# pangenome/allwave

Measured on AMD Instinct MI355X. Metric: aligned base-pairs/sec (whole node) + PAF lines/sec, all-pairs 10 kbp, higher is better.
Workload: dtype int16

## Files before the change

allwave_amd/csrc/biwfa_device.hpp:

```cpp


#include <hip/hip_runtime.h>
#include <stdint.h>
#include <limits.h>

#include "range_span.hpp"
#include "twin_base.hpp"
#include "row_reuse.hpp"

#ifndef AWV_NS
#define AWV_NS awv
#endif
#ifndef AWV_WG
#define AWV_WG 64
#endif
namespace AWV_NS {

constexpr int WG = AWV_WG;
constexpr int MAX_SCOPE = 126;
constexpr int MAX_RING = 256;
constexpr int NCOMP = 5;
constexpr int32_t OFF_NULL = INT32_MIN / 2;
constexpr int32_t NULLISH = INT32_MIN / 4;
constexpr int32_t NULL16 = -16384;
#ifdef AWV_WIDE16
constexpr bool WENC = true;
#else
constexpr bool WENC = false;
#endif
enum { C_M = 0, C_I1 = 1, C_I2 = 2, C_D1 = 3, C_D2 = 4 };
constexpr int FALLBACK_MIN_SCORE = 250;
constexpr int FALLBACK_MIN_LENGTH = 100;
constexpr int STACK_CAP = 48;
constexpr int EV_STACK_WORDS = (STACK_CAP * 32 + 3) / 4 + 16;
constexpr int EV_TWIN_WORDS = MAX_SCOPE * NCOMP;
constexpr int SUB16_MAX_LEN = 32760;
#ifndef AWV_WAVES_PER_SIMD
#define AWV_WAVES_PER_SIMD 4
#endif
constexpr int WAVES_PER_SIMD = AWV_WAVES_PER_SIMD;
constexpr int STATIC_LDS_RESERVE = 1024;
constexpr int COL_PAD = 576;

constexpr int ST_OK = 0, ST_CAPACITY = 1, ST_INTERNAL = 2, ST_MAX_STEPS = 3, ST_ABOVE_BOUND = 4;
constexpr int ST_TWIN_REDO = 64;

struct DevPenalties {
  int x, o1, e1, o2, e2, two_piece, scope;
};

struct DevResult {
  int32_t status, penalty, score;
  uint32_t cigar_len;
  uint64_t cigar_off;
  int32_t num_matches, num_mismatches, num_ins, num_del, q_end, t_end;
};

enum { STAT_CELLS = 0, STAT_EXTEND, STAT_BREAKPOINTS, STAT_BASE, STAT_OVERLAP, STAT_ALIGNED_BP, STAT_PAIRS,
       STAT_T_TOTAL, STAT_T_BI_COMPUTE, STAT_T_BI_BARRIER, STAT_T_BI_FINALIZE, STAT_T_OVERLAP, STAT_T_BASE_STEPS,
       STAT_T_BACKTRACE, STAT_T_EMIT, STAT_N_PASSES,
       STAT_T_CR_LOAD, STAT_T_CR_ALU, STAT_T_CR_EXTEND, STAT_T_CR_STORE, STAT_T_CR_REDUCE, STAT_RESTARTS, STAT_MULTI_CELLS, STAT_WIN_SINGLE, STAT_WIN_MULTI, STAT_WIN_BASE, STAT_WIN_BASE_MULTI,
       STAT_CLK_CYCLES, STAT_CLK_TICKS,
       STAT_DEEP_CELLS,
       STAT_N,
       STAT_TWIN_UNITS = STAT_N, STAT_TWIN_SHARED, STAT_TWIN_SOLO, STAT_TWIN_NONMIRROR,
       STAT_REUSE_CELLS, STAT_REUSE_SEARCHES,
       STAT_N_DEV };

#ifdef AWV_PROF
#define PROF_DRAIN() __builtin_amdgcn_s_waitcnt(0)
#define PROF_NOW() __builtin_readcyclecounter()
#define PROF_ADD(slot, t0) do { if (threadIdx.x == 0) lstats[slot] += __builtin_readcyclecounter() - (t0); } while (0)
#define PROF_INC(slot) do { if (threadIdx.x == 0) lstats[slot] += 1; } while (0)
#define PROF_ADD_L(slot, t0) do { if (threadIdx.x == 0) sh.prof[(slot) - STAT_T_CR_LOAD] += __builtin_readcyclecounter() - (t0); } while (0)
#else
#define PROF_ADD_L(slot, t0) do { (void)(t0); } while (0)
#define PROF_DRAIN() do { } while (0)
#define PROF_NOW() 0ULL
#define PROF_ADD(slot, t0) do { (void)(t0); } while (0)
#define PROF_INC(slot) do { } while (0)
#endif

struct KParams {
  const uint8_t* seq[4];
  const uint64_t* seq_off;
  const int32_t* seq_len;
  const uint32_t* seq2[2];
  const uint64_t* seq2_off;
  const uint8_t* seq2_ok;
  const int32_t* pair_q;
  const int32_t* pair_t;
  const int32_t* pair_rc;
  long long npairs;
  DevPenalties pen;
  int ring;
  int chain_max;
  int multi_T;
  int deep_passes;
  int sub16;
  int wcap;
  void* ring_mem;
  size_t ring_slot_stride;
  int lds_meta_bytes;
  int lds_seq_bytes;
  int sb_cap;
  int wb_cap;
  void* hist_mem;
  size_t hist_slot_stride;
  size_t hist_meta_offset;
  uint32_t* ev_mem;
  size_t ev_slot_stride;
  uint8_t* cigar;
  const uint64_t* cigar_off;
  DevResult* results;
  unsigned long long* work_counter;
  unsigned long long* stats;
  int score_only;
  int max_penalty;
  const int32_t* pair_max_penalty;
  const int32_t* unit_first;
  const int32_t* unit_twin;
  int twin_levels;
  int twin_base;
};
constexpr int RR_DESC_WORDS = 4;

struct RowMeta { int lo, hi; };
constexpr int K_BIG = 1 << 28;
#define ROW_EMPTY RowMeta{K_BIG, -K_BIG}
struct Acc { int hull_lo[NCOMP]; int hull_hi[NCOMP]; int maxak; int oob; int reach; };
struct Task { int pb, pe, tb, te, cb, ce, score_remaining, known; };
constexpr int TM_A = 0, TM_B = 1, TM_SHARED = 2;
constexpr bool TWIN_BUILD = WG == 64 && !WENC;
constexpr int TWIN_MAGIC = 0x7477696e;
__device__ __forceinline__ int twin_comp(int c) { return c == 0 ? 0 : (c <= 2 ? c + 2 : c - 2); }
struct Breakpoint { int score, sf, sr, kf, kr, off_f, off_r, comp; };
static_assert(sizeof(Task) == 32 && sizeof(Breakpoint) == 32, "stack entry / twin record size");

__device__ __forceinline__ int s_min(int a, int b) { int r; asm("s_min_i32 %0, %1, %2" : "=s"(r) : "s"(a), "s"(b) : "scc"); return r; }
__device__ __forceinline__ int s_max(int a, int b) { int r; asm("s_max_i32 %0, %1, %2" : "=s"(r) : "s"(a), "s"(b) : "scc"); return r; }
__device__ __forceinline__ int s_add(int a, int b) { int r; asm("s_add_i32 %0, %1, %2" : "=s"(r) : "s"(a), "s"(b) : "scc"); return r; }

struct alignas(4) RowMeta16 { int16_t lo, hi; };
template <typename OffT> struct MetaTraits;
#ifdef AWV_WIDE16
template <> struct MetaTraits<int16_t> { typedef RowMeta Stored; };
#else
template <> struct MetaTraits<int16_t> { typedef RowMeta16 Stored; };
#endif
template <> struct MetaTraits<int32_t> { typedef RowMeta Stored; };
__device__ __forceinline__ RowMeta meta_load(const RowMeta16* p) {
  const RowMeta16 m = *p;
  return m.lo > m.hi ? ROW_EMPTY : RowMeta{m.lo, m.hi};
}
__device__ __forceinline__ RowMeta meta_load(const RowMeta* p) { return *p; }
__device__ __forceinline__ void meta_store(RowMeta16* p, const RowMeta& m) {
  *p = m.lo > m.hi ? RowMeta16{1, 0} : RowMeta16{(int16_t)m.lo, (int16_t)m.hi};
}
__device__ __forceinline__ void meta_store_scalar(RowMeta16* p, int lo, int hi) {
  int w;
  asm("s_pack_ll_b32_b16 %0, %1, %2\n\ts_cmp_gt_i32 %1, %2\n\ts_cselect_b32 %0, 1, %0" : "=&s"(w) : "s"(lo), "s"(hi) : "scc");
  *reinterpret_cast<int*>(p) = w;
}
__device__ __forceinline__ void meta_store_scalar(RowMeta* p, int lo, int hi) {
  int l, h;
  asm("s_cmp_gt_i32 %2, %3\n\ts_cselect_b32 %0, %4, %2\n\ts_cselect_b32 %1, %5, %3" : "=&s"(l), "=&s"(h) : "s"(lo), "s"(hi), "s"(K_BIG), "s"(-K_BIG) : "scc");
  *p = RowMeta{l, h};
}
__device__ __forceinline__ void meta_store(RowMeta* p, const RowMeta& m) { *p = m; }

template <typename OffT>
struct Lds {
  typename MetaTraits<OffT>::Stored* ring_meta;
  int* bi_A;
  int* bi_oob;
  int* firstk;
  uint32_t* seq;
  RowMeta* meta_log;
};
struct PassCtx {
  unsigned long long ring_mem;
  unsigned long long ring_bytes;
  unsigned long long P[2], T[2];
  int ring, wcap;
  int x, o1, e1, o2, e2;
// ... 3701 lines not shown
  cx.tb_abs = uni(pc.tb_abs);
  Lds<OffT> lds;
  typedef typename MetaTraits<OffT>::Stored MetaStored;
  lds.ring_meta = reinterpret_cast<MetaStored*>(dyn_smem);
  lds.bi_A = reinterpret_cast<int*>(lds.ring_meta + 2 * NCOMP * kp.ring);
  lds.bi_oob = lds.bi_A + 2 * kp.ring;
  lds.firstk = lds.bi_oob + 2 * kp.ring;
  lds.seq = reinterpret_cast<uint32_t*>(dyn_smem + kp.lds_meta_bytes);
  lds.meta_log = nullptr;
  void* ring_mem = (void*)(__attribute__((address_space(1))) char*)(uintptr_t)uni64(pc.ring_mem);
  const rsrc_t ring_rs = make_rsrc(ring_mem, kp.ring_slot_stride);
  __syncthreads();
  Breakpoint bp;
  const int rc = find_breakpoint_reuse<P2, OffT>(kp, sh, lds, cx, ring_mem, ring_rs, cb, ce, score_remaining, known, attempt, bp, lstats);
  if (threadIdx.x == 0) sh.bp_out = bp;
  __syncthreads();
  return rc;
}

template <bool P2, typename OffT, typename... PairSpan>
__global__ __launch_bounds__(WG, WAVES_PER_SIMD) void biwfa_align_kernel(KParams kp, PairSpan... pair_span_arg) {
  constexpr bool RANGES = sizeof...(PairSpan) > 0;
  static_assert(sizeof...(PairSpan) <= 1, "one optional argument: const awvr::Span*");
  __shared__ Shared sh;
  __shared__ unsigned long long lstats[STAT_N];
  static_assert(sizeof(Shared) + sizeof(unsigned long long) * STAT_N <= STATIC_LDS_RESERVE, "static LDS reserve");
  extern __shared__ __attribute__((aligned(16))) unsigned char dyn_smem[];
  Lds<OffT> lds;
  typedef typename MetaTraits<OffT>::Stored MetaStored;
  lds.ring_meta = reinterpret_cast<MetaStored*>(dyn_smem);
  lds.bi_A = reinterpret_cast<int*>(lds.ring_meta + 2 * NCOMP * kp.ring);
  lds.bi_oob = lds.bi_A + 2 * kp.ring;
  lds.firstk = lds.bi_oob + 2 * kp.ring;
  lds.seq = reinterpret_cast<uint32_t*>(dyn_smem + kp.lds_meta_bytes);
  const int tid = cold_tid();
  const DevPenalties& pn = kp.pen;
  void* ring_mem = (char*)kp.ring_mem + (size_t)blockIdx.x * kp.ring_slot_stride;
  void* hist = (char*)kp.hist_mem + (size_t)blockIdx.x * kp.hist_slot_stride;
  uint32_t* events = kp.ev_mem + (size_t)blockIdx.x * kp.ev_slot_stride;
  Task* const stack = reinterpret_cast<Task*>(events + kp.wcap);
  const rsrc_t hist_rs = make_rsrc(hist, kp.hist_slot_stride);
  lds.meta_log = reinterpret_cast<RowMeta*>((char*)hist + kp.hist_meta_offset);
  if (tid < STAT_N) lstats[tid] = 0;
#ifdef AWV_PROF
  if (tid < 5) sh.prof[tid] = 0;
#endif
  const unsigned long long clk_c0 = __builtin_amdgcn_s_memtime(), clk_r0 = __builtin_amdgcn_s_memrealtime();
  if (tid < 16) sh.chain_maxak[tid >> 3][tid & 7] = 0;
  __syncthreads();
  constexpr bool TWINS = TWIN_BUILD && !RANGES && sizeof(OffT) == 2;
  if constexpr (TWINS) {
  const unsigned long long rr_mem = kp.stats[STAT_N_DEV], rr_stride = kp.stats[STAT_N_DEV + 1], rr_pt = kp.stats[STAT_N_DEV + 2];
  const int rr_passes = uni((int)(unsigned)rr_pt), rr_T = uni((int)(rr_pt >> 32)), rr_nid = uni((int)kp.stats[STAT_N_DEV + 3]);
  int* const rr_hdr = rr_mem != 0 && rr_passes > 0 && pn.scope * NCOMP >= RRS_WORDS ? (int*)((char*)(uintptr_t)rr_mem + (size_t)blockIdx.x * (size_t)rr_stride) : nullptr;
  if (rr_hdr != nullptr && tid < awvrr::H_WORDS) rr_hdr[tid] = 0;
  for (;;) {
    if (tid == 0) {
      sh.cur_pair = (long long)atomicAdd(kp.work_counter, 1ULL);
      sh.win_single = sh.win_multi = sh.win_base = sh.win_base_multi = 0;
    }
    __syncthreads();
    const long long unit = ((long long)uni((int)(sh.cur_pair >> 32)) << 32) | (unsigned)uni((int)sh.cur_pair);
    if (unit >= kp.npairs) break;
    long long pair = unit, pair_b = -1;
    if constexpr (TWINS) {
      if (kp.unit_first) {
        pair = uni(kp.unit_first[unit]);
        pair_b = uni(kp.unit_twin[unit]);
      }
    }
    const int qi = kp.pair_q[pair], ti = kp.pair_t[pair];
    const int qv = kp.pair_rc[pair] ? 2 : 0;
    const uint64_t qoff = kp.seq_off[qi], toff = kp.seq_off[ti];
    int plenT = kp.seq_len[qi], tlenT = kp.seq_len[ti];
    const uint8_t* Pf = kp.seq[qv] + qoff;
    const uint8_t* Pr = kp.seq[qv + 1] + qoff;
    const uint8_t* Tf = kp.seq[0] + toff;
    const uint8_t* Tr = kp.seq[1] + toff;
    const int qok = (kp.seq2_ok[qi] >> (qv ? 1 : 0)) & 1, tok = kp.seq2_ok[ti] & 1;
    gwords_t Pw = nullptr, Tw = nullptr;
    if (qok && tok && kp.lds_seq_bytes > 0) {
      Pw = (gwords_t)(uintptr_t)(kp.seq2[qv ? 1 : 0] + kp.seq2_off[qi]);
      Tw = (gwords_t)(uintptr_t)(kp.seq2[0] + kp.seq2_off[ti]);
    }
    int tw_shared = 0, tw_solo = 0, tw_nonmirror = 0;
    int run_mode = TWINS && pair_b >= 0 ? TM_SHARED : TM_A;
    int todo = 0;
    for (;;) {
    const unsigned long long tt0 = PROF_NOW();
    int cur = TM_A;
    Emit em, em_o;
    em.cig = kp.score_only ? nullptr : kp.cigar + kp.cigar_off[pair];
    em.n = 0;
    em.cnt[0] = em.cnt[1] = em.cnt[2] = em.cnt[3] = 0;
    em_o = em;
    if (pair_b >= 0 && !kp.score_only) em_o.cig = kp.cigar + kp.cigar_off[pair_b];
    int status = ST_OK;
    int penalty = -1, penalty_o = -1;
    bool top = true, top_o = true;
    auto face = [&](int o) {
      if (cur == o) return;
      cur = o;
      { const uint8_t* x = Pf; Pf = Tf; Tf = x; }
      { const uint8_t* x = Pr; Pr = Tr; Tr = x; }
      { const gwords_t x = Pw; Pw = Tw; Tw = x; }
      { const int x = plenT; plenT = tlenT; tlenT = x; }
// ... 52 lines not shown
      cx.T[0] = to_global(Tf + t.tb);
      cx.P[1] = to_global(Pr + (plenT - t.pe));
      cx.T[1] = to_global(Tr + (tlenT - t.te));
      cx.kmin[0] = cx.kmin[1] = 0;
      cx.wcols = 0;
      cx.Pw = Pw;
      cx.Tw = Tw;
      cx.pb_abs = t.pb;
      cx.tb_abs = t.tb;
      stage_sequences<OffT>(kp, lds, cx);
      do_base = t.score_remaining <= FALLBACK_MIN_SCORE;
      if (!do_base) {
        int rc = BP_OK;
        for (int attempt = 0; attempt < AWV_RESTART_ATTEMPTS; ++attempt) {
          if (tid == 0) {
            PassCtx& pc = sh.pctx;
            pc.ring_mem = (unsigned long long)(uintptr_t)ring_mem;
            pc.ring_bytes = (unsigned long long)kp.ring_slot_stride;
            pc.P[0] = (unsigned long long)(uintptr_t)cx.P[0];
            pc.P[1] = (unsigned long long)(uintptr_t)cx.P[1];
            pc.T[0] = (unsigned long long)(uintptr_t)cx.T[0];
            pc.T[1] = (unsigned long long)(uintptr_t)cx.T[1];
            pc.Pw = (unsigned long long)(uintptr_t)cx.Pw;
            pc.Tw = (unsigned long long)(uintptr_t)cx.Tw;
            pc.ring = kp.ring;
            pc.wcap = kp.wcap;
            pc.x = pn.x; pc.o1 = pn.o1; pc.e1 = pn.e1; pc.o2 = pn.o2; pc.e2 = pn.e2;
            pc.lds_meta_bytes = kp.lds_meta_bytes;
            pc.lds_seq_bytes = kp.lds_seq_bytes;
            pc.chain_max = kp.chain_max;
            pc.multi_T = kp.multi_T;
            pc.deep_passes = kp.deep_passes;
            pc.max_penalty = kp.pair_max_penalty ? kp.pair_max_penalty[pair] : kp.max_penalty;
            pc.plen = plen; pc.tlen = tlen;
            pc.seq_mode = cx.seq_mode; pc.p_w0 = cx.p_w0; pc.t_w0 = cx.t_w0; pc.p_bit = cx.p_bit; pc.t_bit = cx.t_bit;
            pc.pb_abs = cx.pb_abs; pc.tb_abs = cx.tb_abs;
            const unsigned long long tab = (unsigned long long)(uintptr_t)(events + kp.wcap + EV_STACK_WORDS);
            sh.bp_out.comp = mode == TM_SHARED && !kp.score_only ? TWIN_MAGIC : 0;
            sh.bp_out.off_f = (int)(unsigned)tab;
            sh.bp_out.off_r = (int)(unsigned)(tab >> 32);
            if (mode == TM_SHARED)
              reinterpret_cast<Breakpoint*>(dyn_smem + kp.lds_meta_bytes - sizeof(Breakpoint))->score = INT_MAX;
          }
          __syncthreads();
          if constexpr (sizeof(OffT) == 4 && !WENC) {
            if (kp.sub16 != 0 && max(plen, tlen) < SUB16_MAX_LEN)
              rc = uni(find_breakpoint_fn<P2, int16_t>((unsigned)(uintptr_t)&sh, (unsigned)(uintptr_t)lds.ring_meta, (unsigned)(uintptr_t)lstats,
                                                       t.cb, t.ce, t.score_remaining, t.known, attempt | 0x100));
            else
              rc = uni(find_breakpoint_fn<P2, OffT>((unsigned)(uintptr_t)&sh, (unsigned)(uintptr_t)lds.ring_meta, (unsigned)(uintptr_t)lstats,
                                                    t.cb, t.ce, t.score_remaining, t.known, attempt));
          } else if (rr_hdr != nullptr) {
            int part = 0;
            if (t.score_remaining == INT_MAX) part = RR_RECORD;
            else if (rr_bv >= 0 && (mode == rr_mode || (rr_mode == TM_SHARED && mode == TM_A))) {
              if (t.pb == 0 && t.tb == 0 && t.pe == rr_bv && t.te == rr_bh && t.cb == C_M && t.ce == rr_comp) part = RR_FWD;
              else if (t.pb == rr_bv && t.tb == rr_bh && t.pe == plenT && t.te == tlenT && t.cb == rr_comp && t.ce == C_M) part = RR_REV;
            }
            if (tid == 0) {
              const unsigned long long ra = (unsigned long long)(uintptr_t)rr_hdr;
              lds.firstk[RRS_ARCH_LO] = (int)(unsigned)ra;
              lds.firstk[RRS_ARCH_HI] = (int)(unsigned)(ra >> 32);
              lds.firstk[RRS_PASSES] = rr_passes;
              lds.firstk[RRS_T] = rr_T;
              lds.firstk[RRS_NID] = rr_nid;
              lds.firstk[RRS_PART] = part;
              if (part == RR_RECORD) rr_hdr[awvrr::H_NPASS] = 0;
            }
            __syncthreads();
            rc = uni(find_breakpoint_fn_reuse<P2, OffT>((unsigned)(uintptr_t)&sh, (unsigned)(uintptr_t)lds.ring_meta, (unsigned)(uintptr_t)lstats,
                                                        t.cb, t.ce, t.score_remaining, t.known, attempt));
          } else {
            rc = uni(find_breakpoint_fn<P2, OffT>((unsigned)(uintptr_t)&sh, (unsigned)(uintptr_t)lds.ring_meta, (unsigned)(uintptr_t)lstats,
                                                  t.cb, t.ce, t.score_remaining, t.known, attempt));
          }
          if (rc == BP_OK) {
            bp.score = uni(sh.bp_out.score); bp.sf = uni(sh.bp_out.sf); bp.sr = uni(sh.bp_out.sr); bp.kf = uni(sh.bp_out.kf);
            bp.kr = uni(sh.bp_out.kr); bp.off_f = uni(sh.bp_out.off_f); bp.off_r = uni(sh.bp_out.off_r); bp.comp = uni(sh.bp_out.comp);
            if (mode == TM_SHARED && !kp.score_only) {
              const Breakpoint* rec = reinterpret_cast<const Breakpoint*>(dyn_smem + kp.lds_meta_bytes - sizeof(Breakpoint));
              bq.score = uni(rec->score); bq.sf = uni(rec->sf); bq.sr = uni(rec->sr); bq.kf = uni(rec->kf);
              bq.off_f = uni(rec->off_f); bq.comp = uni(rec->comp);
            }
          }
          if (rc != BP_RESTART) break;
          if (tid == 0) lstats[STAT_RESTARTS] += 1;
        }
        if (TWINS && pair_b >= 0 && run_mode == TM_SHARED) {
          if (mode == TM_SHARED) ++tw_shared;
          else ++tw_solo;
        }
        if (rc == BP_END_REACHED) {
          if (mode == TM_SHARED) split = true;
          else do_base = true;
        }
        else if (rc == BP_ABOVE_BOUND) { status = ST_ABOVE_BOUND; break; }
        else if (rc != BP_OK) { status = rc; break; }
      }
      }
      bool shared_base = false;
      if (split && kp.twin_base != 0) {
        if (tlen == 0 || plen == 0) {
          const int n = max(plen, tlen);
          const int pen_gap = n > 0 ? min(pn.o1 + n * pn.e1, P2 ? pn.o2 + n * pn.e2 : INT_MAX) : 0;
          emit_run(em, tlen == 0 ? 'D' : 'I', n);
          emit_run(em_o, plen == 0 ? 'D' : 'I', n);
          if (top) penalty = pen_gap;
          if (top_o) penalty_o = pen_gap;
          top = top_o = false;
          continue;
        }
        if (t.score_remaining <= FALLBACK_MIN_SCORE) {
          cx.plen = plen;
          cx.tlen = tlen;
          cx.P[0] = to_global(Pf + t.pb);
          cx.T[0] = to_global(Tf + t.tb);
          cx.P[1] = to_global(Pr + (plenT - t.pe));
          cx.T[1] = to_global(Tr + (tlenT - t.te));
          cx.kmin[0] = cx.kmin[1] = 0;
          cx.wcols = 0;
          cx.Pw = Pw;
          cx.Tw = Tw;
          cx.pb_abs = t.pb;
          cx.tb_abs = t.tb;
// ... 80 lines not shown
      else if (failed_in == TM_B) { write_b = true; todo = 1; }
      else { write_a = true; todo = 2; }
    }
    const int pair_bound = kp.pair_max_penalty ? kp.pair_max_penalty[pair] : kp.max_penalty;
    if (status == ST_OK && penalty > pair_bound) {
      status = ST_ABOVE_BOUND;
      em.cnt[0] = em.cnt[1] = em.cnt[2] = em.cnt[3] = 0;
    }
    if (tid == 0) {
      auto record = [&](long long pi, const Emit& e, int pen, int qlen) {
        DevResult r;
        r.status = status;
        r.penalty = status == ST_OK ? pen : status == ST_ABOVE_BOUND ? pair_bound + 1 : 0;
        r.score = -r.penalty;
        r.cigar_len = status == ST_OK && !kp.score_only ? (uint32_t)e.n : 0u;
        r.cigar_off = kp.score_only ? 0 : kp.cigar_off[pi];
        r.num_matches = e.cnt[0];
        r.num_mismatches = e.cnt[1];
        r.num_ins = e.cnt[2];
        r.num_del = e.cnt[3];
        r.q_end = e.cnt[0] + e.cnt[1] + e.cnt[3];
        r.t_end = e.cnt[0] + e.cnt[1] + e.cnt[2];
        kp.results[pi] = r;
        if (status == ST_OK) {
          lstats[STAT_ALIGNED_BP] += (unsigned long long)qlen;
          lstats[STAT_PAIRS] += 1;
        }
      };
      if constexpr (RANGES) {
        record(pair, em, penalty, (pair_span_arg, ...)[pair].pe - (pair_span_arg, ...)[pair].pb);
      } else {
        if (write_a) record(pair, em, penalty, plenT);
        if (TWINS && write_b) record(pair_b, em_o, penalty_o, tlenT);
      }
      PROF_ADD(STAT_T_TOTAL, tt0);
      lstats[STAT_WIN_SINGLE] += sh.win_single; lstats[STAT_WIN_MULTI] += sh.win_multi; lstats[STAT_WIN_BASE] += sh.win_base; lstats[STAT_WIN_BASE_MULTI] += sh.win_base_multi;
      sh.win_single = sh.win_multi = sh.win_base = sh.win_base_multi = 0;
    }
    __syncthreads();
    if (!TWINS || !todo) break;
    run_mode = (todo & 1) ? TM_A : TM_B;
    todo &= ~(1 << run_mode);
    }
    if (TWINS && pair_b >= 0 && tid == 0) {
      atomicAdd(&kp.stats[STAT_TWIN_UNITS], 1ULL);
      atomicAdd(&kp.stats[STAT_TWIN_SHARED], (unsigned long long)tw_shared);
      atomicAdd(&kp.stats[STAT_TWIN_SOLO], (unsigned long long)tw_solo);
      atomicAdd(&kp.stats[STAT_TWIN_NONMIRROR], (unsigned long long)tw_nonmirror);
    }
  }
  if (rr_hdr != nullptr && tid == 0) {
    const unsigned long long rcells = __hip_atomic_load((unsigned long long*)(rr_hdr + awvrr::H_RCELLS), __ATOMIC_RELAXED, __HIP_MEMORY_SCOPE_AGENT);
    const int rsearch = __hip_atomic_load(rr_hdr + awvrr::H_RSEARCH, __ATOMIC_RELAXED, __HIP_MEMORY_SCOPE_AGENT);
    if (rcells) atomicAdd(&kp.stats[STAT_REUSE_CELLS], rcells);
    if (rsearch) atomicAdd(&kp.stats[STAT_REUSE_SEARCHES], (unsigned long long)rsearch);
  }
  } else {
  for (;;) {
    if (tid == 0) {
      sh.cur_pair = (long long)atomicAdd(kp.work_counter, 1ULL);
      sh.error = 0;
      sh.win_single = sh.win_multi = sh.win_base = sh.win_base_multi = 0;
    }
    __syncthreads();
    const long long pair = ((long long)uni((int)(sh.cur_pair >> 32)) << 32) | (unsigned)uni((int)sh.cur_pair);
    if (pair >= kp.npairs) break;
    const int qi = kp.pair_q[pair], ti = kp.pair_t[pair];
    const int qv = kp.pair_rc[pair] ? 2 : 0;
    const uint64_t qoff = kp.seq_off[qi], toff = kp.seq_off[ti];
    const int plenT = kp.seq_len[qi], tlenT = kp.seq_len[ti];
    const uint8_t* Pf = kp.seq[qv] + qoff;
    const uint8_t* Pr = kp.seq[qv + 1] + qoff;
    const uint8_t* Tf = kp.seq[0] + toff;
    const uint8_t* Tr = kp.seq[1] + toff;
    const int qok = (kp.seq2_ok[qi] >> (qv ? 1 : 0)) & 1, tok = kp.seq2_ok[ti] & 1;
    gwords_t Pw = nullptr, Tw = nullptr;
    if (qok && tok && kp.lds_seq_bytes > 0) {
      Pw = (gwords_t)(uintptr_t)(kp.seq2[qv ? 1 : 0] + kp.seq2_off[qi]);
      Tw = (gwords_t)(uintptr_t)(kp.seq2[0] + kp.seq2_off[ti]);
    }
    const unsigned long long tt0 = PROF_NOW();
    Emit em;
    em.cig = kp.score_only ? nullptr : kp.cigar + kp.cigar_off[pair];
    em.n = 0;
    em.cnt[0] = em.cnt[1] = em.cnt[2] = em.cnt[3] = 0;
    int status = ST_OK;
    int penalty = -1;
    int sp = 0;
    if constexpr (RANGES) {
      if (tid == 0) {
        const awvr::Span top = (pair_span_arg, ...)[pair];
        const bool min_length = max(top.pe - top.pb, top.te - top.tb) <= FALLBACK_MIN_LENGTH;
        stack[0] = Task{top.pb, top.pe, top.tb, top.te, C_M, C_M, min_length ? 0 : INT_MAX, INT_MAX};
      }
    } else if (tid == 0) {
      const bool min_length = max(plenT, tlenT) <= FALLBACK_MIN_LENGTH;
      stack[0] = Task{0, plenT, 0, tlenT, C_M, C_M, min_length ? 0 : INT_MAX, INT_MAX};
    }
    sp = 1;
    __syncthreads();
    bool top = true;
    while (sp > 0 && status == ST_OK) {
      Task t = stack[sp - 1];
      t.pb = uni(t.pb); t.pe = uni(t.pe); t.tb = uni(t.tb); t.te = uni(t.te);
      t.cb = uni(t.cb); t.ce = uni(t.ce); t.score_remaining = uni(t.score_remaining); t.known = uni(t.known);
      --sp;
      __syncthreads();
      const int plen = t.pe - t.pb, tlen = t.te - t.tb;
// ... 145 lines not shown
```

allwave_amd/csrc/engine.hip:

```cpp
#include "allwave_hip.h"
#include "host_errors.hpp"
#include "planner_device.hpp"
#include "verify_device.hpp"
#include "clip_device.hpp"
#include "split_device.hpp"
#include "normalize_device.hpp"
#include "encode_device.hpp"
#include "cs_device.hpp"
#include "coverage_device.hpp"
#include "variants_device.hpp"
#include "lift_device.hpp"
#include "msa_device.hpp"
#include "kernels_awv.hpp"
#define AWV_NS awv
#define AWV_WG 64
#include "biwfa_device.hpp"
#undef AWV_NS
#undef AWV_WG
#define AWV_NS awvw
#define AWV_WG 256
#include "biwfa_device.hpp"
#undef AWV_NS
#undef AWV_WG
#define AWV_NS awvx
// ... 516 lines not shown
    const awvb::Entry& en = ge[(size_t)tp.first[u]];
    const uint64_t cost = awvb::pair_cost(en.ql, en.tl);
    return tp.twin[u] >= 0 ? 2 * cost : cost;
  };
  std::stable_sort(uo.begin(), uo.end(), [&](size_t a, size_t b) { return ucost(a) > ucost(b); });
  st.hufirst.resize(uo.size());
  st.hutwin.resize(uo.size());
  for (size_t u = 0; u < uo.size(); ++u) {
    st.hufirst[u] = tp.first[uo[u]];
    st.hutwin[u] = tp.twin[uo[u]];
  }
  nunits = (int64_t)uo.size();
  if (int rc = e->d_unit_first.reserve((size_t)nunits)) return rc;
  if (int rc = e->d_unit_twin.reserve((size_t)nunits)) return rc;
  AWV_TRY(hipMemcpyAsync(e->d_unit_first.p, st.hufirst.data(), (size_t)nunits * 4, hipMemcpyHostToDevice, e->stream));
  AWV_TRY(hipMemcpyAsync(e->d_unit_twin.p, st.hutwin.data(), (size_t)nunits * 4, hipMemcpyHostToDevice, e->stream));
  return AWV_OK;
}

int upload_group(AlignCall& c, const std::vector<awvb::Entry>& ge, const awvb::RowPlan& rp, int64_t& nunits) {
  awv_engine* e = c.e;
  awv_engine::HostStage& st = e->stage;
  const AlignRequest& rq = c.rq;
  const size_t m = ge.size();
  st.hq.resize(m); st.ht.resize(m); st.hrc.resize(m); st.hoff.resize(m);
  for (size_t i = 0; i < m; ++i) {
    st.hq[i] = ge[i].q; st.ht[i] = ge[i].t; st.hrc[i] = ge[i].rc; st.hoff[i] = ge[i].off;
  }
  AWV_TRY(hipEventRecord(e->ev0, e->stream));
  AWV_TRY(hipMemcpyAsync(e->d_pair_q.p, st.hq.data(), m * 4, hipMemcpyHostToDevice, e->stream));
  AWV_TRY(hipMemcpyAsync(e->d_pair_t.p, st.ht.data(), m * 4, hipMemcpyHostToDevice, e->stream));
  AWV_TRY(hipMemcpyAsync(e->d_pair_rc.p, st.hrc.data(), m * 4, hipMemcpyHostToDevice, e->stream));
  AWV_TRY(hipMemcpyAsync(e->d_cigar_off.p, st.hoff.data(), m * 8, hipMemcpyHostToDevice, e->stream));
  if (rq.pair_bound) {
    st.hbound.resize(m);
    for (size_t i = 0; i < m; ++i) st.hbound[i] = rq.pair_bound[c.first + ge[i].batch_index];
    if (int rc = e->d_pair_bound.reserve(m)) return rc;
    AWV_TRY(hipMemcpyAsync(e->d_pair_bound.p, st.hbound.data(), m * 4, hipMemcpyHostToDevice, e->stream));
  }
  if (rq.spans) {
    st.hspan.resize(m);
    for (size_t i = 0; i < m; ++i) st.hspan[i] = rq.spans[c.first + ge[i].batch_index];
    if (int rc = e->d_pair_span.reserve(m)) return rc;
    AWV_TRY(hipMemcpyAsync(e->d_pair_span.p, st.hspan.data(), m * sizeof(awvr::Span), hipMemcpyHostToDevice, e->stream));
  }
  nunits = (int64_t)m;
  if (rp.twin_here)
    if (int rc = upload_twin_units(c, ge, nunits)) return rc;
  AWV_TRY(hipMemsetAsync(e->d_counters.p, 0, (1 + awv::STAT_N_DEV + awv::RR_DESC_WORDS) * sizeof(unsigned long long), e->stream));
  if (c.reuse.passes > 0) {
    st.hreuse[0] = (unsigned long long)(uintptr_t)e->reuse_mem.p;
    st.hreuse[1] = (unsigned long long)c.reuse.bytes();
    st.hreuse[2] = (unsigned long long)(unsigned)c.reuse.passes | ((unsigned long long)(unsigned)c.reuse.T << 32);
    st.hreuse[3] = (unsigned long long)c.reuse.nid;
    AWV_TRY(hipMemcpyAsync(e->d_counters.p + 1 + awv::STAT_N_DEV, st.hreuse, sizeof(st.hreuse), hipMemcpyHostToDevice, e->stream));
  }
  return timer_stop(c, c.h2d_ms);
}

awv::KParams fill_kparams(const AlignCall& c, const awvb::RowPlan& rp, int wc, int64_t nunits) {
  const awv_engine* e = c.e;
  const SeqSet& s = c.s;
  const bool narrow = rp.width != 1;
  awv::KParams kp{};
  for (int v = 0; v < 4; ++v) kp.seq[v] = s.d_seq[v].p;
  kp.seq_off = s.d_off.p;
  kp.seq_len = s.d_len.p;
  kp.seq2[0] = s.d_seq2[0].p;
  kp.seq2[1] = s.d_seq2[1].p;
  kp.seq2_off = s.d_off2.p;
  kp.seq2_ok = s.d_ok2.p;
  kp.pair_q = e->d_pair_q.p;
  kp.pair_t = e->d_pair_t.p;
  kp.pair_rc = e->d_pair_rc.p;
  kp.npairs = nunits;
  kp.unit_first = rp.twin_here ? e->d_unit_first.p : nullptr;
  kp.unit_twin = rp.twin_here ? e->d_unit_twin.p : nullptr;
  kp.twin_levels = (e->cfg.flags & AWV_F_TWIN_TOP_ONLY) ? 1 : INT_MAX;
  kp.twin_base = (e->cfg.flags & AWV_F_NO_TWIN_BASE) ? 0 : 1;
  kp.pen = awv::DevPenalties{c.pp.x, c.pp.o1, c.pp.e1, c.pp.o2, c.pp.e2, c.pp.two_piece, c.pp.scope};
  kp.ring = c.pp.ring;
  kp.multi_T = narrow ? c.pp.multi_T : (std::min(c.pp.multi_T, awv::TMAX32) >= 2 ? std::min(c.pp.multi_T, awv::TMAX32) : 0);
  kp.deep_passes = (kp.multi_T > 0 && !(e->cfg.flags & AWV_F_NO_DEEP)) ? 1 : 0;
  kp.sub16 = (e->cfg.flags & AWV_F_FORCE_INT32) ? 0 : 1;
  kp.chain_max = narrow ? c.pp.chain_max : (awv::TMAX32 == awv::TMAX ? std::min(c.pp.chain_max, 3) : 1);
  kp.wcap = wc;
  kp.ring_mem = e->ring_mem.p;
  kp.ring_slot_stride = rp.ring_stride(wc);
  kp.lds_meta_bytes = (int)rp.lds_meta;
  kp.lds_seq_bytes = (int)rp.lds_seq;
  kp.sb_cap = c.pp.sb_cap;
  kp.wb_cap = c.pp.wb_cap;
  kp.hist_mem = e->hist_mem.p;
  kp.hist_slot_stride = rp.hist_stride;
  kp.hist_meta_offset = rp.hist_rows;
  kp.ev_mem = e->ev_mem.p;
  kp.ev_slot_stride = rp.ev_stride(wc);
  kp.cigar = e->d_cigar.p;
  kp.cigar_off = e->d_cigar_off.p;
  kp.results = e->d_results.p;
  kp.work_counter = e->d_counters.p;
  kp.stats = e->d_counters.p + 1;
  kp.score_only = c.rq.score_only ? 1 : 0;
  kp.max_penalty = c.rq.max_penalty;
  kp.pair_max_penalty = c.rq.pair_bound ? e->d_pair_bound.p : nullptr;
  return kp;
}
// ... 208 lines not shown
    if (rc != 0) return fail(AWV_ERR_SINK, "sink callback returned " + std::to_string(rc));
    c.lap("sink returned");
    return AWV_OK;
  }
  c.runner.res.swap(c.hres);
  c.runner.cig.swap(c.e->h_cigar);
  c.runner.cs.swap(c.e->h_cs);
  const awv_result* rp = c.runner.res.data();
  const uint8_t* cp = want_cigar ? c.runner.cig.data() : nullptr;
  const uint8_t* xp = want_cigar && with_cs ? c.runner.cs.data() : nullptr;
  const int64_t f0 = c.first, n0 = c.n;
  SinkRunner* rn = &c.runner;
  try {
    c.runner.th = std::thread([rn, sink, user, f0, n0, rp, cp, xp]() { rn->rc = sink(user, f0, n0, rp, cp, xp); });
    c.lap("sink handed off");
  } catch (const std::exception&) {
    const int rc = sink(user, f0, n0, rp, cp, xp);
    if (rc != 0) return fail(AWV_ERR_SINK, "sink callback returned " + std::to_string(rc));
  }
  return AWV_OK;
}

void publish_stats(AlignCall& c) {
  using namespace awv;
  awv_engine* e = c.e;
  const unsigned long long* stat_tot = c.stat_tot;
  e->stats.kernel_ms = c.kernel_ms;
  e->stats.h2d_ms = c.h2d_ms;
  e->stats.d2h_ms = c.d2h_ms;
  e->stats.launches = c.launches;
  e->stats.cell_steps = stat_tot[STAT_CELLS];
  e->stats.extend_steps = stat_tot[STAT_EXTEND];
  e->stats.n_breakpoints = stat_tot[STAT_BREAKPOINTS];
  e->stats.n_base = stat_tot[STAT_BASE];
  e->stats.overlap_scans = stat_tot[STAT_OVERLAP];
  e->stats.aligned_bp = stat_tot[STAT_ALIGNED_BP];
  e->stats.pairs_completed = stat_tot[STAT_PAIRS];
  e->stats.scratch_bytes = e->ring_mem.bytes() + e->hist_mem.bytes() + e->ev_mem.bytes() + e->reuse_mem.bytes();
  for (int i = 0; i < 14; ++i) e->stats.prof[i] = stat_tot[STAT_T_TOTAL + i];
  e->stats.restarts = stat_tot[STAT_RESTARTS];
  e->stats.multi_cell_steps = stat_tot[STAT_MULTI_CELLS];
  e->stats.windows[0] = stat_tot[STAT_WIN_SINGLE];
  e->stats.windows[1] = stat_tot[STAT_WIN_MULTI];
  e->stats.windows[2] = stat_tot[STAT_WIN_BASE];
  e->stats.windows[3] = stat_tot[STAT_WIN_BASE_MULTI];
  e->stats.clock_cycles = stat_tot[STAT_CLK_CYCLES];
  e->stats.clock_ticks = stat_tot[STAT_CLK_TICKS];
  e->stats.clock_tick_khz = (uint64_t)e->wall_clock_khz;
  e->stats.deep_cell_steps = stat_tot[STAT_DEEP_CELLS];
  for (int i = 0; i < 4; ++i) e->twin_stats[i] = stat_tot[STAT_TWIN_UNITS + i];
#if !defined(AWV_PROF) && !defined(AWV_DIAG)
  e->stats.prof[12] = stat_tot[STAT_REUSE_CELLS];
  e->stats.prof[13] = stat_tot[STAT_REUSE_SEARCHES];
#endif
}

int align_core(awv_engine* e, SeqSet& s, const awv_penalties* pen, const AlignRequest& rq) {
  AlignCall c{e, s, pen, rq};
  c.pp = awvb::plan_penalties(LIMITS, pen, e->cfg.flags);
  if (c.pp.code != AWV_OK && !c.pp.late) return fail(c.pp.code, c.pp.message);
  AWV_TRY(hipSetDevice(e->device));
  e->stats = awv_stats{};
  for (uint64_t& v : e->twin_stats) v = 0;
  c.norm = rq.score_only ? AWV_NORM_OFF : e->norm_mode;
  if (rq.npairs == 0) return AWV_OK;
  if (c.pp.code != AWV_OK) return fail(c.pp.code, c.pp.message);
  c.cfg = awvb::Config{e->cfg.flags, e->num_cus, e->cfg.workgroups, (int64_t)e->cfg.max_scratch_bytes, e->cfg.first_row_cols};
  c.max_batch = e->cfg.max_batch_pairs > 0 ? e->cfg.max_batch_pairs : (int64_t)1 << 20;
  c.max_arena = e->cfg.max_arena_bytes > 0 ? (uint64_t)e->cfg.max_arena_bytes : (uint64_t)8 << 30;
  c.twin_ok = rq.max_penalty == INT_MAX && !rq.pair_bound && !rq.spans && !rq.cout && !(e->cfg.flags & (AWV_F_NO_TWIN | AWV_F_NO_RERUN));
  read_knobs(c);
  for (; c.first < rq.npairs; c.first += c.n) {
    const bool skewed = carve_and_order(c);
    if (int rc = reserve_batch_buffers(c)) return rc;
    if (int rc = run_groups(c, skewed)) return rc;
    c.lap("results on host");
    if (int rc = run_record_steps(c)) return rc;
    if (int rc = copy_cigars_back(c)) return rc;
    if (int rc = deliver(c)) return rc;
  }
  publish_stats(c);
  return AWV_OK;
}

int require_sequences(const awv_engine* e, int64_t n, const char* who) {
  if (e->seqs.n == 0 && n > 0) return fail(AWV_ERR_STATE, std::string(who) + " before set_sequences");
  return AWV_OK;
}
int32_t norm_bound(int32_t b) { return b < 0 || b >= (1 << 30) ? INT_MAX : b; }
const int32_t* normalized_bounds(const int32_t* bounds, int64_t n, std::vector<int32_t>& store) {
  if (!bounds || n <= 0) return nullptr;
  store.resize((size_t)n);
  for (int64_t i = 0; i < n; ++i) store[(size_t)i] = norm_bound(bounds[i]);
  return store.data();
}
int split_ranges(const SeqSet& s, const awv_range_pair* ranges, int64_t n, std::vector<awv_pair>& pairs, std::vector<awvr::Span>& spans,
                 const char* who) {
  pairs.resize((size_t)n);
  spans.resize((size_t)n);
  for (int64_t i = 0; i < n; ++i)
    if (!awvr::split_range(s.len.data(), s.n, ranges[i], pairs[(size_t)i], spans[(size_t)i]))
      return fail(AWV_ERR_ARG, std::string(who) + ": range " + std::to_string(i) + " names a sequence index or an interval out of range");
  return AWV_OK;
}
int check_clip_args(const awv_clip_result* cout, int32_t match_bonus) {
  if (!cout) return fail(AWV_ERR_ARG, "align_clipped: null cout");
// ... 465 lines not shown
```

allwave_amd/csrc/row_reuse.hpp:

```cpp
#pragma once
#include <stddef.h>
#include <stdint.h>

#if defined(__HIPCC__) || defined(__CUDACC__)
#define AWVRR_HD __host__ __device__ inline
#else
#define AWVRR_HD inline
#endif

namespace awvrr {

constexpr int NCOMP = 5;
enum { H_NPASS = 0,
       H_KMIN0 = 1,
       H_KMIN1 = 2,
       H_RCELLS = 4,
       H_RSEARCH = 6,
       H_WORDS = 16 };
enum { P_MAXAK = 0,
       P_CELLS = 1,
       P_BOXH = 2,
       P_BOXV = 3,
       P_WORDS = 4 };

struct Layout {
  int passes, T, nid, cols;
  AWVRR_HD int rows_per_pass() const { return T + nid; }
  AWVRR_HD int scores() const { return passes * T; }
  AWVRR_HD int reach() const { return scores(); }
  AWVRR_HD size_t table_off() const { return (size_t)H_WORDS * 4; }
  AWVRR_HD size_t table_index(int dir, int pass) const { return ((size_t)dir * passes + pass) * P_WORDS; }
  AWVRR_HD size_t meta_off() const { return table_off() + (size_t)2 * passes * P_WORDS * 4; }
  AWVRR_HD size_t meta_index(int dir, int s, int c) const { return ((size_t)dir * scores() + (s - 1)) * NCOMP + c; }
  AWVRR_HD size_t rows_off() const { return (meta_off() + (size_t)2 * scores() * NCOMP * 4 + 15) & ~(size_t)15; }
  AWVRR_HD size_t row_index(int dir, int pass, int r) const { return ((size_t)dir * passes + pass) * rows_per_pass() + r; }
  AWVRR_HD size_t row_off(int dir, int pass, int r) const { return rows_off() + row_index(dir, pass, r) * cols * 2; }
  AWVRR_HD size_t bytes() const { return (rows_off() + (size_t)2 * passes * rows_per_pass() * cols * 2 + 255) & ~(size_t)255; }
};

AWVRR_HD int cols_for(int scores) { return (2 * (scores + 8) + 8 + 3) & ~3; }
AWVRR_HD Layout make_layout(int passes, int T, int nid) { return Layout{passes, T, nid, cols_for(passes * T)}; }

AWVRR_HD int first_col(const Layout& l, int kmin) { return (-(l.reach() + 8) - kmin) & ~3; }
AWVRR_HD bool hull_fits(const Layout& l, int lo, int hi) { return lo > hi || (lo >= -l.reach() && hi <= l.reach()); }
AWVRR_HD int pass_of(const Layout& l, int s) { return (s - 1) / l.T; }
AWVRR_HD int row_of(const Layout& l, int s) { return (s - 1) % l.T; }
AWVRR_HD int id_row(const Layout& l, int e1, int e2, int comp, int j) {
  const int base = comp == 1 ? 0 : comp == 3 ? e1 : comp == 2 ? 2 * e1 : 2 * e1 + e2;
  const int e = (comp == 1 || comp == 3) ? e1 : e2;
  return l.T + base + (e - 1 - j);
}

AWVRR_HD bool box_ok(int boxh, int boxv, int plen, int tlen) { return boxh <= 2 * tlen && boxv <= 2 * plen; }

AWVRR_HD int pass_for(const Layout& l, int npass, int sc, int Tc) {
  if (Tc != l.T || sc < 0 || sc % l.T != 0) return -1;
  const int p = sc / l.T;
  return p < npass && p < l.passes ? p : -1;
}

inline int plan_passes(int maxsum, int T, int nid, long long nslots, unsigned long long avail) {
  if (T < 2 || nslots <= 0) return 0;
  int passes = (maxsum / 28 < 4096 ? maxsum / 28 : 4096) / T;
  while (passes >= 4 && (unsigned long long)make_layout(passes, T, nid).bytes() * (unsigned long long)nslots > avail) passes = passes * 3 / 4;
  return passes >= 4 ? passes : 0;
}

}
```

allwave_amd/ffi.py:

```python
import ctypes as C
import os

import numpy as np

_HERE = os.path.dirname(os.path.abspath(__file__))
LIB_PATH = os.environ.get("AWV_HIP_LIB") or os.path.join(_HERE, "liballwave_hip.so")

AWV_OK = 0
AWV_ERR_NO_DEVICE = -1
AWV_ERR_ARG = -3
AWV_ERR_STATE = -6
AWV_ERR_SINK = -7
AWV_ST_COMPLETED = 0
AWV_ST_CAPACITY = 1
AWV_ST_ABOVE_BOUND = 4
AWV_F_KEEP_ON_DEVICE = 1
AWV_F_FORCE_INT32 = 2
AWV_F_NO_PACKED_SEQ = 4
AWV_F_ONE_WAVE = 8
AWV_F_FOUR_WAVES = 16
AWV_F_NO_ARENA_PROBE = 32
AWV_F_SINGLE_STEP = 64
AWV_F_NO_CHAIN = 128
AWV_F_NO_WIDE16 = 256
AWV_F_NO_DEEP = 512
AWV_F_NO_RERUN = 1024
AWV_F_NO_TWIN = 2048
AWV_F_TWIN_TOP_ONLY = 4096
AWV_F_NO_TWIN_BASE = 8192
AWV_F_NO_ROW_REUSE = 16384
AWV_ORIENT_FORWARD = 0
AWV_ORIENT_REVERSE = 1
AWV_ORIENT_UNDECIDED = 2
AWV_ORIENT_BY_BOUND = 0
AWV_ORIENT_BY_EDITS = 1
AWV_ORIENT_FULL = 1
AWV_ORIENT_SKIP_RATIO = 8
AWV_ORIENT_NO_EDITS = 2 ** 64 - 1
AWV_ORIENT_HI_NONE = 2 ** 31 - 1
AWV_VF_OK = 0
AWV_VF_SKIPPED = 1
AWV_VF_BAD_OP = 2
AWV_VF_OVERRUN = 3
AWV_VF_M_DIFFERS = 4
AWV_VF_X_EQUAL = 5
AWV_VF_SHORT = 6
AWV_VF_COUNTS = 7
AWV_VF_PENALTY = 8
AWV_CL_OK = 0
AWV_CL_SKIPPED = 1
AWV_CL_EMPTY = 2
AWV_CL_BAD_OP = 3
AWV_CLIP_MAX_BONUS = 32767
AWV_NORM_OFF = 0
AWV_NORM_LEFT = 1
AWV_NORM_RIGHT = 2
AWV_NM_OK = 0
AWV_NM_SKIPPED = 1
AWV_NM_BAD_OP = 2
AWV_NM_LENGTHS = 3
AWV_CS_SHORT = 1
AWV_CS_LONG = 2
AWV_CST_OK = 0
AWV_CST_SKIPPED = 1
AWV_CST_BAD_OP = 2
AWV_CST_LENGTHS = 3
AWV_COV_TARGET = 1
AWV_COV_QUERY = 2
AWV_COV_BOTH = 3
AWV_CV_OK = 0
AWV_CV_SKIPPED = 1
AWV_CV_BAD_OP = 2
AWV_CV_LENGTHS = 3
AWV_VAR_SNV = 0
AWV_VAR_DEL = 1
AWV_VAR_INS = 2
AWV_VAR_HASH_BASE = 0x1b873593a5c1f2e7
AWV_VAR_HASH_MOD = (1 << 61) - 1
AWV_VR_OK = 0
AWV_VR_SKIPPED = 1
AWV_VR_BAD_OP = 2
AWV_VR_LENGTHS = 3
AWV_VTAB_EVENTS = 0
# ... 1177 lines not shown
```

include/allwave_hip.h:

```cpp
#ifndef ALLWAVE_HIP_H
#define ALLWAVE_HIP_H

#include <stddef.h>
#include <stdint.h>

#ifdef __cplusplus
extern "C" {
#endif

#define AWV_ABI_VERSION 3

#define AWV_OK 0
#define AWV_ERR_NO_DEVICE (-1)
#define AWV_ERR_HIP (-2)
#define AWV_ERR_ARG (-3)
#define AWV_ERR_PENALTIES (-4)
#define AWV_ERR_OOM (-5)
#define AWV_ERR_STATE (-6)
#define AWV_ERR_SINK (-7)

#define AWV_ST_COMPLETED 0
#define AWV_ST_CAPACITY 1
#define AWV_ST_INTERNAL 2
#define AWV_ST_MAX_STEPS 3
#define AWV_ST_ABOVE_BOUND 4

typedef struct awv_engine awv_engine;

typedef struct {
  int32_t device;
  int32_t workgroups;
  int64_t max_batch_pairs;
  int64_t max_arena_bytes;
  int32_t flags;
  int32_t first_row_cols;
  int64_t max_scratch_bytes;
} awv_engine_config;

#define AWV_F_KEEP_ON_DEVICE 1
#define AWV_F_NO_ARENA_PROBE 32
#define AWV_F_NO_RERUN 1024
#define AWV_F_FORCE_INT32 2
#define AWV_F_NO_WIDE16 256
#define AWV_F_NO_PACKED_SEQ 4
#define AWV_F_ONE_WAVE 8
#define AWV_F_FOUR_WAVES 16
#define AWV_F_NO_CHAIN 128
#define AWV_F_NO_DEEP 512
#define AWV_F_SINGLE_STEP 64
#define AWV_F_NO_TWIN 2048
#define AWV_F_TWIN_TOP_ONLY 4096
#define AWV_F_NO_TWIN_BASE 8192
#define AWV_F_NO_ROW_REUSE 16384

typedef struct {
  int32_t match;
  int32_t mismatch;
  int32_t gap_open1;
  int32_t gap_ext1;
  int32_t gap_open2;
  int32_t gap_ext2;
  int32_t two_piece;
} awv_penalties;

typedef struct {
  int32_t q_idx;
  int32_t t_idx;
  int32_t q_revcomp;
} awv_pair;

typedef struct {
  int32_t status;
  int32_t penalty;
  int32_t score;
  uint32_t cigar_len;
  uint64_t cigar_off;
  int32_t num_matches;
  int32_t num_mismatches;
  int32_t num_ins;
  int32_t num_del;
  int32_t q_end;
  int32_t t_end;
} awv_result;

typedef int (*awv_sink)(void* user, int64_t first, int64_t n, const awv_result* results,
                        const uint8_t* cigar_arena);

typedef struct {
  double kernel_ms;
  double h2d_ms, d2h_ms;
  uint64_t launches;
  uint64_t cell_steps;
  uint64_t extend_steps;
  uint64_t n_breakpoints;
  uint64_t n_base;
  uint64_t overlap_scans;
  uint64_t aligned_bp;
  uint64_t pairs_completed;
  uint64_t scratch_bytes;
  uint64_t prof[14];
  uint64_t restarts;
  uint64_t multi_cell_steps;
  uint64_t windows[4];
  uint64_t clock_cycles, clock_ticks;
  uint64_t clock_tick_khz;
  uint64_t deep_cell_steps;
// ... 497 lines not shown
```

Baseline: 788.1 million.

## Extend row reuse to deeper BiWFA recursion tasks anchored at sequence ends

Result: faster. 825.0 million, median of 6 (+4.7%).

```diff
diff --git a/allwave_amd/csrc/biwfa_device.hpp b/allwave_amd/csrc/biwfa_device.hpp
--- a/allwave_amd/csrc/biwfa_device.hpp
+++ b/allwave_amd/csrc/biwfa_device.hpp
@@ -64,7 +64,7 @@
        STAT_DEEP_CELLS,
        STAT_N,
        STAT_TWIN_UNITS = STAT_N, STAT_TWIN_SHARED, STAT_TWIN_SOLO, STAT_TWIN_NONMIRROR,
-       STAT_REUSE_CELLS, STAT_REUSE_SEARCHES,
+       STAT_REUSE_CELLS, STAT_REUSE_SEARCHES, STAT_REUSE_DEEP_CELLS, STAT_REUSE_DEEP_SEARCHES,
        STAT_N_DEV };
 
 #ifdef AWV_PROF
@@ -131,6 +131,7 @@
 struct Acc { int hull_lo[NCOMP]; int hull_hi[NCOMP]; int maxak; int oob; int reach; };
 struct Task { int pb, pe, tb, te, cb, ce, score_remaining, known; };
 constexpr int TM_A = 0, TM_B = 1, TM_SHARED = 2;
+static_assert(TM_A == awvrr::FR_A && TM_B == awvrr::FR_B && TM_SHARED == awvrr::FR_SHARED, "row_reuse.hpp names the same frames");
 constexpr bool TWIN_BUILD = WG == 64 && !WENC;
 constexpr int TWIN_MAGIC = 0x7477696e;
 __device__ __forceinline__ int twin_comp(int c) { return c == 0 ? 0 : (c <= 2 ? c + 2 : c - 2); }
@@ -3938,6 +3939,7 @@
   if constexpr (TWINS) {
   const unsigned long long rr_mem = kp.stats[STAT_N_DEV], rr_stride = kp.stats[STAT_N_DEV + 1], rr_pt = kp.stats[STAT_N_DEV + 2];
   const int rr_passes = uni((int)(unsigned)rr_pt), rr_T = uni((int)(rr_pt >> 32)), rr_nid = uni((int)kp.stats[STAT_N_DEV + 3]);
+  const int rr_levels = uni((int)(kp.stats[STAT_N_DEV + 3] >> 32));
   int* const rr_hdr = rr_mem != 0 && rr_passes > 0 && pn.scope * NCOMP >= RRS_WORDS ? (int*)((char*)(uintptr_t)rr_mem + (size_t)blockIdx.x * (size_t)rr_stride) : nullptr;
   if (rr_hdr != nullptr && tid < awvrr::H_WORDS) rr_hdr[tid] = 0;
   for (;;) {
@@ -4096,10 +4098,13 @@
                                                     t.cb, t.ce, t.score_remaining, t.known, attempt));
           } else if (rr_hdr != nullptr) {
             int part = 0;
+            bool below_one = false;
             if (t.score_remaining == INT_MAX) part = RR_RECORD;
-            else if (rr_bv >= 0 && (mode == rr_mode || (rr_mode == TM_SHARED && mode == TM_A))) {
-              if (t.pb == 0 && t.tb == 0 && t.pe == rr_bv && t.te == rr_bh && t.cb == C_M && t.ce == rr_comp) part = RR_FWD;
-              else if (t.pb == rr_bv && t.tb == rr_bh && t.pe == plenT && t.te == tlenT && t.cb == rr_comp && t.ce == C_M) part = RR_REV;
+            else if (rr_bv >= 0 && awvrr::frame_ok(rr_mode, mode)) {
+              bool level1;
+              const int tdir = awvrr::take_dir(awvrr::RootId{plenT, tlenT, rr_bv, rr_bh, rr_comp}, awvrr::TaskId{t.pb, t.pe, t.tb, t.te, t.cb, t.ce}, rr_levels, &level1);
+              part = tdir == 0 ? RR_FWD : tdir == 1 ? RR_REV : 0;
+              below_one = tdir >= 0 && !level1;
             }
             if (tid == 0) {
               const unsigned long long ra = (unsigned long long)(uintptr_t)rr_hdr;
@@ -4110,10 +4115,24 @@
               lds.firstk[RRS_NID] = rr_nid;
               lds.firstk[RRS_PART] = part;
               if (part == RR_RECORD) rr_hdr[awvrr::H_NPASS] = 0;
+              rr_hdr[awvrr::H_DNOW] = below_one ? 1 : 0;
+              if (below_one) {
+                *(unsigned long long*)(rr_hdr + awvrr::H_DMARK) = __hip_atomic_load((unsigned long long*)(rr_hdr + awvrr::H_RCELLS), __ATOMIC_RELAXED, __HIP_MEMORY_SCOPE_AGENT);
+                rr_hdr[awvrr::H_DSMARK] = __hip_atomic_load(rr_hdr + awvrr::H_RSEARCH, __ATOMIC_RELAXED, __HIP_MEMORY_SCOPE_AGENT);
+              }
             }
             __syncthreads();
             rc = uni(find_breakpoint_fn_reuse<P2, OffT>((unsigned)(uintptr_t)&sh, (unsigned)(uintptr_t)lds.ring_meta, (unsigned)(uintptr_t)lstats,
                                                         t.cb, t.ce, t.score_remaining, t.known, attempt));
+            if (tid == 0 && __hip_atomic_load(rr_hdr + awvrr::H_DNOW, __ATOMIC_RELAXED, __HIP_MEMORY_SCOPE_AGENT) != 0) {
+              const unsigned long long now = __hip_atomic_load((unsigned long long*)(rr_hdr + awvrr::H_RCELLS), __ATOMIC_RELAXED, __HIP_MEMORY_SCOPE_AGENT);
+              const unsigned long long mark = __hip_atomic_load((unsigned long long*)(rr_hdr + awvrr::H_DMARK), __ATOMIC_RELAXED, __HIP_MEMORY_SCOPE_AGENT);
+              const unsigned long long dc = __hip_atomic_load((unsigned long long*)(rr_hdr + awvrr::H_DCELLS), __ATOMIC_RELAXED, __HIP_MEMORY_SCOPE_AGENT);
+              *(unsigned long long*)(rr_hdr + awvrr::H_DCELLS) = dc + (now - mark);
+              const int snow = __hip_atomic_load(rr_hdr + awvrr::H_RSEARCH, __ATOMIC_RELAXED, __HIP_MEMORY_SCOPE_AGENT);
+              const int smark = __hip_atomic_load(rr_hdr + awvrr::H_DSMARK, __ATOMIC_RELAXED, __HIP_MEMORY_SCOPE_AGENT);
+              rr_hdr[awvrr::H_DSEARCH] = __hip_atomic_load(rr_hdr + awvrr::H_DSEARCH, __ATOMIC_RELAXED, __HIP_MEMORY_SCOPE_AGENT) + (snow - smark);
+            }
           } else {
             rc = uni(find_breakpoint_fn<P2, OffT>((unsigned)(uintptr_t)&sh, (unsigned)(uintptr_t)lds.ring_meta, (unsigned)(uintptr_t)lstats,
                                                   t.cb, t.ce, t.score_remaining, t.known, attempt));
@@ -4300,8 +4319,12 @@
   if (rr_hdr != nullptr && tid == 0) {
     const unsigned long long rcells = __hip_atomic_load((unsigned long long*)(rr_hdr + awvrr::H_RCELLS), __ATOMIC_RELAXED, __HIP_MEMORY_SCOPE_AGENT);
     const int rsearch = __hip_atomic_load(rr_hdr + awvrr::H_RSEARCH, __ATOMIC_RELAXED, __HIP_MEMORY_SCOPE_AGENT);
-    if (rcells) atomicAdd(&kp.stats[STAT_REUSE_CELLS], rcells);
-    if (rsearch) atomicAdd(&kp.stats[STAT_REUSE_SEARCHES], (unsigned long long)rsearch);
+    const unsigned long long dcells = __hip_atomic_load((unsigned long long*)(rr_hdr + awvrr::H_DCELLS), __ATOMIC_RELAXED, __HIP_MEMORY_SCOPE_AGENT);
+    const int dsearch = __hip_atomic_load(rr_hdr + awvrr::H_DSEARCH, __ATOMIC_RELAXED, __HIP_MEMORY_SCOPE_AGENT);
+    if (rcells - dcells) atomicAdd(&kp.stats[STAT_REUSE_CELLS], rcells - dcells);
+    if (rsearch - dsearch) atomicAdd(&kp.stats[STAT_REUSE_SEARCHES], (unsigned long long)(rsearch - dsearch));
+    if (dcells) atomicAdd(&kp.stats[STAT_REUSE_DEEP_CELLS], dcells);
+    if (dsearch) atomicAdd(&kp.stats[STAT_REUSE_DEEP_SEARCHES], (unsigned long long)dsearch);
   }
   } else {
   for (;;) {
diff --git a/allwave_amd/csrc/engine.hip b/allwave_amd/csrc/engine.hip
--- a/allwave_amd/csrc/engine.hip
+++ b/allwave_amd/csrc/engine.hip
@@ -592,7 +592,7 @@
     st.hreuse[0] = (unsigned long long)(uintptr_t)e->reuse_mem.p;
     st.hreuse[1] = (unsigned long long)c.reuse.bytes();
     st.hreuse[2] = (unsigned long long)(unsigned)c.reuse.passes | ((unsigned long long)(unsigned)c.reuse.T << 32);
-    st.hreuse[3] = (unsigned long long)c.reuse.nid;
+    st.hreuse[3] = (unsigned long long)c.reuse.nid | ((unsigned long long)((e->cfg.flags & AWV_F_ROW_REUSE_LEVEL1) ? awvrr::LV_ONE : awvrr::LV_ALL) << 32);
     AWV_TRY(hipMemcpyAsync(e->d_counters.p + 1 + awv::STAT_N_DEV, st.hreuse, sizeof(st.hreuse), hipMemcpyHostToDevice, e->stream));
   }
   return timer_stop(c, c.h2d_ms);
@@ -907,6 +907,8 @@
 #if !defined(AWV_PROF) && !defined(AWV_DIAG)
   e->stats.prof[12] = stat_tot[STAT_REUSE_CELLS];
   e->stats.prof[13] = stat_tot[STAT_REUSE_SEARCHES];
+  e->stats.prof[10] = stat_tot[STAT_REUSE_DEEP_CELLS];
+  e->stats.prof[11] = stat_tot[STAT_REUSE_DEEP_SEARCHES];
 #endif
 }
 
diff --git a/allwave_amd/csrc/row_reuse.hpp b/allwave_amd/csrc/row_reuse.hpp
--- a/allwave_amd/csrc/row_reuse.hpp
+++ b/allwave_amd/csrc/row_reuse.hpp
@@ -16,6 +16,11 @@
        H_KMIN1 = 2,
        H_RCELLS = 4,
        H_RSEARCH = 6,
+       H_DCELLS = 8,
+       H_DMARK = 10,
+       H_DNOW = 12,
+       H_DSMARK = 13,
+       H_DSEARCH = 14,
        H_WORDS = 16 };
 enum { P_MAXAK = 0,
        P_CELLS = 1,
@@ -59,6 +64,21 @@
   return p < npass && p < l.passes ? p : -1;
 }
 
+struct RootId { int plen, tlen, bv, bh, bcomp; };
+struct TaskId { int pb, pe, tb, te, cb, ce; };
+constexpr int LV_ALL = 0, LV_ONE = 1;
+constexpr int FR_A = 0, FR_B = 1, FR_SHARED = 2;
+AWVRR_HD bool frame_ok(int root_frame, int task_frame) { return task_frame == root_frame || (root_frame == FR_SHARED && task_frame == FR_A); }
+AWVRR_HD int take_dir(const RootId& r, const TaskId& t, int levels, bool* level1) {
+  const bool fwd = t.pb == 0 && t.tb == 0 && t.cb == 0, rev = t.pe == r.plen && t.te == r.tlen && t.ce == 0;
+  *level1 = true;
+  if (fwd && t.pe == r.bv && t.te == r.bh && t.ce == r.bcomp) return 0;
+  if (rev && t.pb == r.bv && t.tb == r.bh && t.cb == r.bcomp) return 1;
+  *level1 = false;
+  if (levels == LV_ONE) return -1;
+  return fwd ? 0 : rev ? 1 : -1;
+}
+
 inline int plan_passes(int maxsum, int T, int nid, long long nslots, unsigned long long avail) {
   if (T < 2 || nslots <= 0) return 0;
   int passes = (maxsum / 28 < 4096 ? maxsum / 28 : 4096) / T;
diff --git a/allwave_amd/ffi.py b/allwave_amd/ffi.py
--- a/allwave_amd/ffi.py
+++ b/allwave_amd/ffi.py
@@ -29,6 +29,7 @@
 AWV_F_TWIN_TOP_ONLY = 4096
 AWV_F_NO_TWIN_BASE = 8192
 AWV_F_NO_ROW_REUSE = 16384
+AWV_F_ROW_REUSE_LEVEL1 = 32768
 AWV_ORIENT_FORWARD = 0
 AWV_ORIENT_REVERSE = 1
 AWV_ORIENT_UNDECIDED = 2
diff --git a/include/allwave_hip.h b/include/allwave_hip.h
--- a/include/allwave_hip.h
+++ b/include/allwave_hip.h
@@ -52,6 +52,7 @@
 #define AWV_F_TWIN_TOP_ONLY 4096
 #define AWV_F_NO_TWIN_BASE 8192
 #define AWV_F_NO_ROW_REUSE 16384
+#define AWV_F_ROW_REUSE_LEVEL1 32768
 
 typedef struct {
   int32_t match;
```
